# ElBaldo1/FastOptSolver

Measured on AMD Instinct MI355X. Metric: fista_iterations_per_second, higher is better.
Workload: dtype f32

## Files before the change

### fastoptsolver_amd/csrc/cluster_pass.hpp

```cpp
#pragma once
#include "batch_trial.hpp"

namespace fos {

constexpr int CP_ROWS = 16;
constexpr int CP_W = 1024;
constexpr int CP_ASTRIDE = CP_W + 4;
constexpr int CP_THREADS = 320;
constexpr int CP_SLOTS = 4;
constexpr int CP_FLAG_STRIDE = 32;
constexpr unsigned CP_SPIN_LIMIT = 1u << 18;
constexpr size_t CP_LDS_BYTES = (size_t)2 * CP_ROWS * CP_ASTRIDE * 4 + 4 * 64 * 16 + 2 * 64 * 16 + 16;

typedef unsigned long long cp_u64;
__device__ inline void cp_store_sc1(cp_u64* p, cp_u64 v) { __hip_atomic_store(p, v, __ATOMIC_RELAXED, __HIP_MEMORY_SCOPE_AGENT); }
__device__ inline cp_u64 cp_load_sc1(const cp_u64* p) { return __hip_atomic_load(p, __ATOMIC_RELAXED, __HIP_MEMORY_SCOPE_AGENT); }
__device__ inline cp_u64 cp_pack(float lo, float hi) { return ((cp_u64)__float_as_uint(hi) << 32) | __float_as_uint(lo); }

template <int CS, int MODE = 0>
__global__ __launch_bounds__(CP_THREADS) void cluster_pass_kernel(const float* __restrict__ A, int64_t lda,
                                                                 const float* __restrict__ b, int64_t m, int n, int n_pad,
                                                                 const float* __restrict__ xp, int64_t rows_per_cluster,
                                                                 int xcd_aware, float* __restrict__ xchg,
                                                                 unsigned* __restrict__ flags, unsigned epoch,
                                                                 float* __restrict__ slabs, int64_t n_stride,
                                                                 int* __restrict__ error) {
  extern __shared__ __attribute__((aligned(16))) char cp_lds[];
  float (*a_s)[CP_ROWS][CP_ASTRIDE] = reinterpret_cast<float (*)[CP_ROWS][CP_ASTRIDE]>(cp_lds);
  f32x4 (*red)[64] = reinterpret_cast<f32x4 (*)[64]>(cp_lds + (size_t)2 * CP_ROWS * CP_ASTRIDE * 4);
  f32x4 (*r_s)[64] = reinterpret_cast<f32x4 (*)[64]>(cp_lds + (size_t)2 * CP_ROWS * CP_ASTRIDE * 4 + 4 * 64 * 16);
  int* abort_s = reinterpret_cast<int*>(cp_lds + (size_t)2 * CP_ROWS * CP_ASTRIDE * 4 + 4 * 64 * 16 + 2 * 64 * 16);

  const int tid = threadIdx.x, lane = tid & 63, wave = tid >> 6;
  const bool mc = wave < 4;
  int cluster, member;
  if (xcd_aware) {
    const int xcd = blockIdx.x % 8, idx = blockIdx.x / 8;
    cluster = xcd + 8 * (idx / CS);
    member = idx % CS;
  } else {
    cluster = blockIdx.x / CS;
    member = blockIdx.x % CS;
  }
  const int col_strip = member * CP_W;
  const int64_t row_lo = (int64_t)cluster * rows_per_cluster;
  const int npanels = (int)(rows_per_cluster / CP_ROWS);
  if (tid == 0) *abort_s = 0;

  f32x4 xr[16];
  f32x4 G[16];
  f32x4 areg[CP_ROWS];
  const int wcol = col_strip + 256 * (wave & 3);
  if (mc) {
#pragma unroll
    for (int s = 0; s < 16; ++s) {
      const int col = wcol + 16 * s;
      const f32x4 v = *reinterpret_cast<const f32x4*>(xp + ((int64_t)((col < n_pad ? col : 0) / 16) * 4 + (lane >> 4)) * 64 +
                                                      (lane & 15) * 4);
      xr[s] = col < n_pad ? v : f32x4{0.f, 0.f, 0.f, 0.f};
      G[s] = f32x4{0.f, 0.f, 0.f, 0.f};
    }
  }
  int lcol = col_strip + 4 * tid;
  if (lcol >= n) lcol = n - 4;
  auto load_tile = [&](int pnl) {
    if ((MODE & 4) && pnl >= 2) return;
    if (pnl >= npanels) pnl = npanels - 1;
#pragma unroll
    for (int u = 0; u < CP_ROWS; ++u) {
      int64_t row = row_lo + (int64_t)pnl * CP_ROWS + u;
      if (row >= m) row = m - 1;
      areg[u] = __builtin_nontemporal_load(reinterpret_cast<const f32x4*>(A + row * lda + lcol));
    }
  };
  auto store_tile = [&](int buf) {
#pragma unroll
    for (int u = 0; u < CP_ROWS; ++u) *reinterpret_cast<f32x4*>(&a_s[buf][u][4 * tid]) = areg[u];
  };

  if (mc) {
    load_tile(0);
    store_tile(0);
    load_tile(1);
  }
  __syncthreads();

  for (int i = 0; i <= npanels; ++i) {
    if (mc) {
      if (i < npanels) {
        const int buf = i & 1;
        f32x4 acc = {0.f, 0.f, 0.f, 0.f}, acc_odd = {0.f, 0.f, 0.f, 0.f};
#pragma unroll
        for (int s = 0; s < ((MODE & 2) ? 1 : 16); ++s) {
          const f32x4 a4 = *reinterpret_cast<const f32x4*>(&a_s[buf][lane & 15][256 * wave + 16 * s + 4 * (lane >> 4)]);
          acc = __builtin_amdgcn_mfma_f32_16x16x4f32(a4.x, xr[s].x, acc, 0, 0, 0);
          acc_odd = __builtin_amdgcn_mfma_f32_16x16x4f32(a4.y, xr[s].y, acc_odd, 0, 0, 0);
          acc = __builtin_amdgcn_mfma_f32_16x16x4f32(a4.z, xr[s].z, acc, 0, 0, 0);
          acc_odd = __builtin_amdgcn_mfma_f32_16x16x4f32(a4.w, xr[s].w, acc_odd, 0, 0, 0);
        }
        red[wave][lane] = acc + acc_odd;
      }
    } else if (i >= 1 && (MODE & 1)) {
      r_s[(i - 1) & 1][lane] = red[0][lane];
    } else if (i >= 1) {
      const int q = i - 1;
      bool ok = true;
      if (lane < CS) {
        const unsigned* f = flags + ((size_t)cluster * CS + lane) * CP_FLAG_STRIDE;
        unsigned spins = 0;
        while ((int)(__hip_atomic_load(f, __ATOMIC_RELAXED, __HIP_MEMORY_SCOPE_AGENT) - epoch) < q + 1) {
          if (++spins > CP_SPIN_LIMIT) { ok = false; break; }
          __builtin_amdgcn_s_sleep(1);
        }
      }
      if (__ballot(!ok) != 0) {
        if (lane == 0) { *abort_s = 1; *error = 1; }
      } else {
        constexpr int GC = CS < 8 ? CS : 8;
        f32x4 r = {0.f, 0.f, 0.f, 0.f};
#pragma unroll 1
        for (int j0 = 0; j0 < CS; j0 += GC) {
          cp_u64 lo[GC], hi[GC];
#pragma unroll
          for (int j = 0; j < GC; ++j) {
            const cp_u64* src = reinterpret_cast<const cp_u64*>(
                xchg + (((size_t)cluster * CP_SLOTS + (q % CP_SLOTS)) * CS + j0 + j) * 256 + lane * 4);
            lo[j] = cp_load_sc1(src);
            hi[j] = cp_load_sc1(src + 1);
          }
#pragma unroll
          for (int j = 0; j < GC; ++j) {
            r.x += __uint_as_float((unsigned)lo[j]); r.y += __uint_as_float((unsigned)(lo[j] >> 32));
            r.z += __uint_as_float((unsigned)hi[j]); r.w += __uint_as_float((unsigned)(hi[j] >> 32));
          }
        }
        const int64_t row0 = row_lo + (int64_t)q * CP_ROWS + 4 * (lane >> 4);
        float rv[4] = {r.x, r.y, r.z, r.w};
#pragma unroll
        for (int c = 0; c < 4; ++c) {
          const int64_t row = row0 + c;
          rv[c] = row < m ? (b != nullptr ? rv[c] - b[row] : rv[c]) : 0.f;
        }
        r_s[q & 1][lane] = f32x4{rv[0], rv[1], rv[2], rv[3]};
      }
    }
    __syncthreads();
    if (*abort_s) break;
    if (mc) {
      if (i >= 1) {
        const int buf = (i - 1) & 1;
        const f32x4 r4 = r_s[(i - 1) & 1][lane];
        const float rc[4] = {r4.x, r4.y, r4.z, r4.w};
#pragma unroll
        for (int c = 0; c < ((MODE & 2) ? 1 : 4); ++c) {
#pragma unroll
          for (int t = 0; t < 16; ++t)
            G[t] = __builtin_amdgcn_mfma_f32_16x16x4f32(rc[c], a_s[buf][4 * (lane >> 4) + c][256 * wave + 16 * t + (lane & 15)],
                                                        G[t], 0, 0, 0);
        }
      }
    } else if (i < npanels && !(MODE & 1)) {
      const f32x4 s = ((red[0][lane] + red[1][lane]) + red[2][lane]) + red[3][lane];
      cp_u64* dst = reinterpret_cast<cp_u64*>(xchg + (((size_t)cluster * CP_SLOTS + (i % CP_SLOTS)) * CS + member) * 256 + lane * 4);
      cp_store_sc1(dst, cp_pack(s.x, s.y));
      cp_store_sc1(dst + 1, cp_pack(s.z, s.w));
      asm volatile("s_waitcnt vmcnt(0)" ::: "memory");
      if (lane == 0)
        __hip_atomic_store(flags + ((size_t)cluster * CS + member) * CP_FLAG_STRIDE, epoch + (unsigned)i + 1u, __ATOMIC_RELAXED,
                           __HIP_MEMORY_SCOPE_AGENT);
    }
    __syncthreads();
    if (mc && i + 1 < npanels) {
      store_tile((i + 1) & 1);
      load_tile(i + 2);
    }
    __syncthreads();
  }

  if (mc && *abort_s == 0) {
#pragma unroll
    for (int t = 0; t < 16; ++t) {
      const int col = wcol + 16 * t + (lane & 15);
      if (col < n) {
        const float gv[4] = {G[t].x, G[t].y, G[t].z, G[t].w};
#pragma unroll
        for (int r = 0; r < 4; ++r) slabs[((int64_t)cluster * BT_NV + 4 * (lane >> 4) + r) * n_stride + col] = gv[r];
      }
    }
  }
}

}
```

### fastoptsolver_amd/csrc/fos_internal.hpp

```cpp
#pragma once
#include <hip/hip_runtime.h>

#include <algorithm>
#include <atomic>
#include <cmath>
#include <cstdio>
#include <cstring>
#include <memory>
#include <string>
#include <chrono>
#include <vector>

#pragma GCC visibility push(default)
#include "../../include/fos.h"
#pragma GCC visibility pop
#include "batch_trial.hpp"
#include "cluster_pass.hpp"
#include "comm.hpp"
#include "gemv_multi.hpp"
#include "gemv_pair.hpp"
#include "gemv_tall.hpp"
#include "gemv_wide.hpp"
#include "gram_batch.hpp"
#include "gram_batch_dd.hpp"
// ... 4 lines not shown
#include "resident_batch.hpp"


namespace fosapi {

extern thread_local std::string g_err;

inline int fail(int code, const std::string& msg) {
  g_err = msg;
  return code;
}
#define HIP_TRY(expr)                                                                                   \
  do {                                                                                                  \
    hipError_t e_ = (expr);                                                                             \
    if (e_ != hipSuccess)                                                                               \
      return fail(FOS_ERR_HIP, std::string(#expr) + ": " + hipGetErrorString(e_));                      \
  } while (0)
#define LAUNCH_CHECK()                                                                                  \
  do {                                                                                                  \
    hipError_t e_ = hipGetLastError();                                                                  \
    if (e_ != hipSuccess) return fail(FOS_ERR_HIP, std::string("kernel launch: ") + hipGetErrorString(e_)); \
  } while (0)

template <class T, bool PINNED = false>
class DevBuf {
 public:
  DevBuf() = default;
  DevBuf(DevBuf&& o) noexcept : ptr_(o.ptr_), bytes_(o.bytes_) { o.ptr_ = nullptr; o.bytes_ = 0; }
  DevBuf& operator=(DevBuf&& o) noexcept {
    if (this != &o) {
      reset();
      std::swap(ptr_, o.ptr_);
      std::swap(bytes_, o.bytes_);
    }
    return *this;
  }
  ~DevBuf() { reset(); }
  void reset() {
    if (ptr_) (void)(PINNED ? hipHostFree(ptr_) : hipFree(ptr_));
    ptr_ = nullptr;
    bytes_ = 0;
  }
  int reserve(size_t count) {
    const size_t need = count * sizeof(T);
    if (ptr_ && need <= bytes_) return FOS_OK;
    reset();
    const hipError_t e = PINNED ? hipHostMalloc(&ptr_, need) : hipMalloc(&ptr_, need);
    if (e != hipSuccess) {
      ptr_ = nullptr;
      return fail(FOS_ERR_HIP, std::string(PINNED ? "hipHostMalloc(" : "hipMalloc(") + std::to_string(need) + " bytes): " +
                                   hipGetErrorString(e));
    }
    bytes_ = need;
    return FOS_OK;
  }
  T* get() const { return ptr_; }
  operator T*() const { return ptr_; }
  T* operator->() const { return ptr_; }

 private:
  T* ptr_ = nullptr;
  size_t bytes_ = 0;
};
template <class T>
using PinnedBuf = DevBuf<T, true>;

using fos::YSource;

typedef void (*FusedLaunch)(const void* A, int64_t lda, const float* b, int64_t m, int n, YSource ys, int64_t rpw,
                            float* slabs, double* rr_part, double* rr2_part, int nwg, hipStream_t st);

typedef void (*FusedLaunchDD)(const void* A, int64_t lda, const float* b, int64_t m, int n, YSource ys, int64_t rpw,
                              double* slabs, double* rr_part, int nwg, hipStream_t st);
struct MenuEntry {
  int dtype, threads, k, r;
  FusedLaunch with_g, resid_only, dual;
  FusedLaunchDD dd;
  FusedLaunch with_g_cb = nullptr, resid_only_cb = nullptr;
  FusedLaunch with_g_il = nullptr, resid_only_il = nullptr, dual_il = nullptr;
};
struct DdEntry { int dtype, threads, k, r; FusedLaunchDD fn; FusedLaunchDD fn_il = nullptr; };
typedef void (*MultiLaunch)(const float* A, int64_t lda, const float* b, int64_t m, int n, fos::MultiY ys, int64_t rpw,
                            float* slabs, double* rr_part, int nwg, hipStream_t st);
}

using fosapi::MenuEntry;
using fosapi::DdEntry;

using fosapi::DevBuf;
using fosapi::PinnedBuf;

struct LbfgsWork {
  int64_t n = 0;
  DevBuf<double> g, g_old, d, x_old, S, Y, vl;
  PinnedBuf<double> host;
  DevBuf<unsigned long long> t_start;
  double ticks_per_ms = 1e5;
  bool pass_stamps = false;
};

struct LbfgsMultiWork {
  int64_t n = 0;
  DevBuf<double> g;
  DevBuf<double> d, x_old, S, Y, vl, rr;
  PinnedBuf<double> host;
  DevBuf<unsigned> count;
  DevBuf<unsigned long long> t_start;
  double ticks_per_ms = 1e5;
};


struct PassPlan {
  int path = 0;
  bool resident = false;
  bool tall = false;
  bool colblock = false;
  int64_t cb_width = 0;
  int64_t slab_stride = 0;
  bool vec4 = false;
  const MenuEntry* entry = nullptr;
  int nwg = 0;
  int nslabs = 0;
  int64_t rows_per_wg = 0;
  int resid_grid = 0;
  DevBuf<float> slabs;
  DevBuf<double> rr_part;
  DevBuf<double> rr2_part;
  DevBuf<double> rvec;
  DevBuf<float> rneg;
  DevBuf<float> zeros;
  void reset() { *this = PassPlan{}; }
};

struct DdPlan {
  bool planned = false;
  const DdEntry* entry = nullptr;
  int nwg = 0;
  int64_t rows_per_wg = 0;
  int two_pass_chunks = 0;
  DevBuf<double> slabs;
  DevBuf<double> rr;
  void reset() { *this = DdPlan{}; }
};

struct MultiPlan {
  bool planned = false;
  int64_t panel_rows = 0;
  int gram_splits = 0;
  int64_t gram_rows_per_split = 0;
  int cp_cs = 0, cp_clusters = 0;
  int64_t cp_rows_per_cluster = 0;
  DevBuf<float> rbuf16;
  DevBuf<float> slabs16;
  DevBuf<float> cp_xchg;
  DevBuf<unsigned> cp_flags;
  DevBuf<int> cp_error;
  void reset() { *this = MultiPlan{}; }
};

struct DdMultiPlan {
  bool planned = false;
  int64_t n_pad = 0, panel_rows = 0, rows_per_split = 0;
  int splits = 0;
  DevBuf<double> xd;
  DevBuf<double> rdd;
  DevBuf<double> slabs;
  DevBuf<double> q_part;
  void reset() { *this = DdMultiPlan{}; }
};

struct CandPlan {
  bool planned = false;
  int64_t n_pad = 0;
  DevBuf<float> xp;
  DevBuf<double> q_part;
  DevBuf<double> bt_out;
  void reset() { *this = CandPlan{}; }
};

struct Scratch {
  DevBuf<float> gbuf_own;
  DevBuf<float> ybuf;
  DevBuf<double> dscal;
  DevBuf<double> part;
  DevBuf<double> lhist;
  DevBuf<float> rcols16;
  DevBuf<float> b16;
  DevBuf<double> mfold;
  DevBuf<double> cr_part;
  DevBuf<unsigned> cr_bar;
  DevBuf<unsigned> fz_bar;
  DevBuf<double> fz_part;
  DevBuf<double> fz_beta;
};

struct fos_problem {
  const void* A = nullptr;
  const float* b = nullptr;
  float* gbuf = nullptr;
  unsigned long long* fz_stamps = nullptr;
  fos_comm* comm = nullptr;
  int64_t m = 0, n = 0, lda = 0;
  int dtype = FOS_F32;
  int loss = FOS_LOSS_SQUARED;
  const float* row_weight = nullptr;
  hipStream_t stream = nullptr;
  int ncu = 256;
  bool col_sharded = false;
  unsigned plan_flags = 0;
  bool allow_resident = true;
  bool il = false;
  int dd_nwg_hint = 0;
  int cp_mode = 0;
  int chip_mode = 0;
  bool fused_on = false;
  unsigned cp_epoch = 1;
  PassPlan pass;
  DdPlan dd;
  MultiPlan multi;
  DdMultiPlan dm;
  CandPlan cand;
  Scratch ws;
  std::unique_ptr<LbfgsWork> lbfgs;
  std::unique_ptr<LbfgsMultiWork> lbfgs_multi;
  int profiling = 0;
  int64_t prof_seq = 0;
  bool prof_open = false;
  std::vector<hipEvent_t> ev_pool;
  size_t ev_used = 0;
  double prof_ms = 0.0;
  int64_t prof_launches = 0;
};

struct fos_fista {
  fos_problem* p = nullptr;
  fos::FistaParams prm{};
  bool host_valid = false;
  double h_t = 1.0, h_beta = 0.0;
  long long h_k = 0;
  DevBuf<double> part2;
  DevBuf<float> ynext;
  bool y_valid = false;
  bool pending = false;
  long long plain_count = 0;
  DevBuf<double> x_cur, x_prev;
  DevBuf<float> dlt;
  DevBuf<fos::FistaScalars> scal;
  bool precise = false;
  DevBuf<double> folded;
  bool tau_on_device = false;
  double* gbuf64 = nullptr;
  DevBuf<double> gbuf64_own;
  DevBuf<double> out5;
  int nupd = 0;
};

namespace fosapi {

const MenuEntry* wide_entry(int dtype);
const MenuEntry* find_entry(int dtype, int threads, int k, int r);
const MenuEntry* default_entry(int dtype, int64_t n);
int epc_of(int dtype);
int grid_1d(int64_t n, int per_block, int cap);
void plan_fused(fos_problem* p, const MenuEntry* e, int nwg_hint);
void apply_plan(fos_problem* p, unsigned flags);
enum PlanInput : unsigned {
  IN_PLAN = 1,
  IN_TUNE = 2,
  IN_TUNE_DD = 4,
  IN_COMM = 8,
  IN_CLUSTER = 16,
};
int invalidate(fos_problem* p, unsigned changed);
int plan_multi_mfma(fos_problem* p);
int ensure_workspace(fos_problem* p);
int ensure_batch_workspace(fos_problem* p);
int ensure_dd(fos_problem* p);
int prof_drain(fos_problem* p);
int prof_mark(fos_problem* p, bool start);
int aligned_vec(fos_problem* p, const float* v, const float** out);
bool batch_supported(const fos_problem* p);
MultiLaunch find_multi(int64_t n, int nv, bool bblock = false);
int pack_candidates(fos_problem* p, const float* X, int nv);
int stage_b16(fos_problem* p, const float* B, int64_t ldb, int nv);
int launch_pass(fos_problem* p, const YSource& ys, const float* b, bool with_g, int* n_rr, bool dual = false,
                double* rr_to = nullptr);
int launch_slab_reduce(fos_problem* p, int n_rr, float* gbuf, double* rr_out, const int* stopped);
int launch_batch_product(fos_problem* p, const void* A, const float* b, int64_t rows_total, int use_b, float* rout, int* nwg_out,
                         const int* stopped = nullptr, bool bblock = false);
bool fold_held_block(const int32_t* held, int nv, fos::FoldHeld* out);
int launch_batch_product_folds(fos_problem* p, const void* A, const float* b, int64_t rows_total, float* rout, int* nwg_out,
                               const uint8_t* fold_of_row, const fos::FoldHeld& held);
int launch_batch_product_logit(fos_problem* p, const void* A, const float* b, int64_t rows_total, float* rout, int* nwg_out,
                               const uint8_t* fold_of_row, const fos::FoldHeld* held);
int launch_batch_product_weighted(fos_problem* p, const void* A, const float* b, int use_b, int64_t rows_total, float* rout,
                                  int* nwg_out, const uint8_t* fold_of_row, const fos::FoldHeld* held, const float* row_weight);
int need_squared(const fos_problem* p, const char* fn);
int launch_residual_batch(fos_problem* p, int use_b, double* out16, const int* stopped = nullptr, const float* b16 = nullptr);
int launch_cluster_pass(fos_problem* p);
int launch_pass_dd(fos_problem* p, const YSource& ys, double alpha2, const double* l2vec, double* out);
int gemv_pair_dd_stamped(fos_problem* p, const double* x, double alpha2, double* grad_rr, unsigned long long* t_stamp, bool* stamped);
int dd_pass_stamps(fos_problem* p, bool* yes);
bool pair_dd_multi_supported(const fos_problem* p);
int pair_dd_multi(fos_problem* p, const fos::DdMultiCols& c, int ncols, unsigned live, double alpha2, const float* b16);
int comm_allreduce(fos_comm* c, void* buf, size_t count, bool f64, hipStream_t st);
int reduce_across(fos_problem* p, void* buf, size_t count, bool f64);

inline int check_batch_items(const char* fn, const fos_batch_item* items, int count, int64_t ld) {
// ... 14 lines not shown
```

### fastoptsolver_amd/csrc/fos_plan.hip

```cpp
#include "fos_internal.hpp"

namespace fosapi {

thread_local std::string g_err;



template <typename T, int THREADS, int K, int R, int MINW, bool WITH_G, int NBUF, bool DUAL, bool DRAIN = false, bool CB = false,
          bool IL = false>
void fused_launch(const void* A, int64_t lda, const float* b, int64_t m, int n, YSource ys, int64_t rpw, float* slabs,
                  double* rr_part, double* rr2_part, int nwg, hipStream_t st) {
  hipLaunchKernelGGL((fos::gemv_pair_kernel<T, THREADS, K, R, true, MINW, WITH_G, NBUF, IL, DUAL, DRAIN, float, false, CB>), dim3(nwg),
                     dim3(THREADS), 0, st, reinterpret_cast<const T*>(A), lda, b, m, n, ys, rpw, slabs, rr_part,
                     rr2_part);
}


template <typename K>
int raise_dynamic_lds(K kernel, size_t bytes, std::atomic<uint64_t>& done) {
  int dev = 0;
  if (hipGetDevice(&dev) != hipSuccess) return FOS_ERR_HIP;
  const uint64_t bit = 1ull << (dev & 63);
  if (done.load(std::memory_order_acquire) & bit) return FOS_OK;
  if (hipFuncSetAttribute(reinterpret_cast<const void*>(kernel), hipFuncAttributeMaxDynamicSharedMemorySize, (int)bytes) !=
// ... 765 lines not shown
constexpr int DM_P1_PER_CU = 2;
int ensure_dd_multi(fos_problem* p) {
  if (p->dm.planned) return FOS_OK;
  const int64_t n = p->n;
  p->dm.n_pad = (n + fos::DM_COLS - 1) / fos::DM_COLS * fos::DM_COLS;
  p->dm.panel_rows = std::min<int64_t>(256 * (int64_t)p->ncu, (p->m + 255) / 256 * 256);
  const int64_t strips = (n + fos::DM_COLS - 1) / fos::DM_COLS;
  int64_t splits = std::max<int64_t>(1, (2 * (int64_t)p->ncu + strips - 1) / strips);
  splits = std::min<int64_t>(splits, std::max<int64_t>(1, p->dm.panel_rows / 256));
  p->dm.rows_per_split = ((p->dm.panel_rows + splits - 1) / splits + fos::DM_ROWS - 1) / fos::DM_ROWS * fos::DM_ROWS;
  p->dm.splits = (int)((p->dm.panel_rows + p->dm.rows_per_split - 1) / p->dm.rows_per_split);
  const int64_t panels = (p->m + p->dm.panel_rows - 1) / p->dm.panel_rows;
  int rc;
  if ((rc = p->dm.xd.reserve((size_t)p->dm.n_pad * fos::BT_NV)) || (rc = p->dm.rdd.reserve((size_t)p->dm.panel_rows * fos::BT_NV)) ||
      (rc = p->dm.slabs.reserve((size_t)p->dm.splits * fos::BT_NV * n)) ||
      (rc = p->dm.q_part.reserve((size_t)panels * DM_P1_PER_CU * p->ncu * fos::BT_NV)))
    return rc;
  p->dm.planned = true;
  return FOS_OK;
}

template <typename T>
int run_pair_dd_multi(fos_problem* p, const fos::DdMultiCols& c, int ncols, unsigned live, double alpha2, const float* b16) {
  const int64_t n = p->n, esz = sizeof(T);
  hipLaunchKernelGGL(fos::xd_pack_kernel, dim3(grid_1d(p->dm.n_pad * fos::BT_NV, 256, 4 * p->ncu)), dim3(256), 0, p->stream, c,
                     live, (int)n, (int)p->dm.n_pad, p->dm.xd);
  LAUNCH_CHECK();
  const int64_t strips = (n + fos::DM_COLS - 1) / fos::DM_COLS;
  int64_t nparts = 0;
  int rc;
  for (int64_t row0 = 0, panel = 0; row0 < p->m; row0 += p->dm.panel_rows, ++panel) {
    const int64_t rows = std::min<int64_t>(p->dm.panel_rows, p->m - row0);
    const T* Ap = reinterpret_cast<const T*>(reinterpret_cast<const char*>(p->A) + (size_t)row0 * p->lda * esz);
    const int64_t ngroups = (rows + fos::DM_ROWS - 1) / fos::DM_ROWS;
    int64_t nwg = std::min<int64_t>(ngroups, DM_P1_PER_CU * (int64_t)p->ncu);
    const int64_t gpw = (ngroups + nwg - 1) / nwg;
    nwg = (ngroups + gpw - 1) / gpw;
    if ((rc = prof_mark(p, true))) return rc;
    hipLaunchKernelGGL(fos::residual_dd_mfma_kernel<T>, dim3((unsigned)nwg), dim3(fos::DM_THREADS), 0, p->stream, Ap, p->lda,
                       b16 + row0 * fos::BT_NV, rows, (int)n, (const double*)p->dm.xd, gpw, p->dm.q_part + nparts * fos::BT_NV,
                       p->dm.rdd);
    LAUNCH_CHECK();
    if ((rc = prof_mark(p, false))) return rc;
    nparts += nwg;
    const dim3 grid((unsigned)strips, (unsigned)p->dm.splits);
    if ((rc = prof_mark(p, true))) return rc;
    if (panel)
      hipLaunchKernelGGL((fos::gram_dd_mfma_kernel<T, true>), grid, dim3(fos::DM_THREADS), 0, p->stream, Ap, p->lda, rows,
                         (int)n, (const double*)p->dm.rdd, p->dm.rows_per_split, p->dm.slabs, n);
    else
      hipLaunchKernelGGL((fos::gram_dd_mfma_kernel<T, false>), grid, dim3(fos::DM_THREADS), 0, p->stream, Ap, p->lda, rows,
                         (int)n, (const double*)p->dm.rdd, p->dm.rows_per_split, p->dm.slabs, n);
    LAUNCH_CHECK();
    if ((rc = prof_mark(p, false))) return rc;
  }
  hipLaunchKernelGGL(fos::pair_dd_multi_finish_kernel, dim3(grid_1d(n, 256, 64), ncols), dim3(256), 0, p->stream,
                     (const double*)p->dm.slabs, p->dm.splits, (int)n, (const double*)p->dm.q_part, (int)nparts, alpha2, c);
  LAUNCH_CHECK();
  return FOS_OK;
}

typedef int (*PairDdMultiRun)(fos_problem*, const fos::DdMultiCols&, int, unsigned, double, const float*);
struct PairDdMultiEntry { int dtype; PairDdMultiRun run; };
const PairDdMultiEntry kPairDdMulti[] = {
    {FOS_F32, run_pair_dd_multi<float>},
    {FOS_BF16, run_pair_dd_multi<fos::bf16_t>},
};

int pair_dd_multi(fos_problem* p, const fos::DdMultiCols& c, int ncols, unsigned live, double alpha2, const float* b16) {
  if (!pair_dd_multi_supported(p))
    return fail(FOS_ERR_UNSUPPORTED, "fos_gemv_pair_dd_multi: no matrix-core pair for this shape (needs the aligned streaming "
                                     "layout, 65..16384 columns, unsharded)");
  if (ncols < 1) return FOS_OK;
  int rc = ensure_dd_multi(p);
  if (rc) return rc;
  for (const auto& e : kPairDdMulti)
    if (e.dtype == p->dtype) return e.run(p, c, ncols, live, alpha2, b16);
  return fail(FOS_ERR_UNSUPPORTED, "fos_gemv_pair_dd_multi: storage type not served");
}

int aligned_vec(fos_problem* p, const float* v, const float** out) {
  if ((reinterpret_cast<uintptr_t>(v) & 15u) == 0) {
    *out = v;
    return FOS_OK;
  }
  HIP_TRY(hipMemcpyAsync(p->ws.ybuf, v, (size_t)p->n * sizeof(float), hipMemcpyDeviceToDevice, p->stream));
  *out = p->ws.ybuf;
  return FOS_OK;
}

bool il_default(const fos_problem* p) {
  const int64_t bytes = p->m * p->n * (p->dtype == FOS_F32 ? 4 : 2);
  return bytes >= (12ll << 30);
}

bool vec_layout(const fos_problem* p) {
  const int epc = epc_of(p->dtype);
  return (p->n % epc == 0) && (p->lda % epc == 0) && ((reinterpret_cast<uintptr_t>(p->A) & 15u) == 0);
}
void plan_resident(fos_problem* p) { p->pass.resident = fos::resident_fits(p->m, p->n) && p->allow_resident && p->comm == nullptr; }
const MenuEntry* colblock_entry(const fos_problem* p, int64_t* width) {
  const int64_t cap = 16384, blocks = (p->n + cap - 1) / cap;
  *width = ((p->n + blocks - 1) / blocks + 63) / 64 * 64;
  const MenuEntry* ce = default_entry(p->dtype, *width);
  return ce && ce->with_g_cb && ce->resid_only_cb ? ce : nullptr;
}
void plan_colblock(fos_problem* p, const MenuEntry* ce, int64_t width) {
  plan_fused(p, ce, 0);
  p->pass.colblock = true;
  p->pass.cb_width = width;
}

void apply_plan(fos_problem* p, unsigned flags) {
  const int64_t n = p->n;
  p->plan_flags = flags;
  p->pass.vec4 = (n % 4 == 0);
  p->allow_resident = !(flags & FOS_PLAN_NO_RESIDENT);
  p->il = (flags & FOS_PLAN_INTERLEAVE) ? true : (flags & FOS_PLAN_NO_INTERLEAVE) ? false : il_default(p);
  plan_resident(p);
  const bool vec_ok = vec_layout(p);
  int64_t cb_width = 0;
  const MenuEntry* e = vec_ok ? default_entry(p->dtype, n) : nullptr;
  if ((n <= fos::TL_MAX_N || (n <= tlr_max_n(p->dtype) && vec_ok)) && !(flags & FOS_PLAN_NO_TALL))
    plan_tall(p, tall_entry(p->dtype, n, p->lda, p->A));
  else if (e) plan_fused(p, e, 0);
  else if (vec_ok && n <= fos::WD_MAX_N && !(flags & FOS_PLAN_NO_WIDE)) plan_fused(p, wide_entry(p->dtype), 0);
  else if (const MenuEntry* ce = (vec_ok && !(flags & FOS_PLAN_NO_COLBLOCK)) ? colblock_entry(p, &cb_width) : nullptr)
    plan_colblock(p, ce, cb_width);
  else plan_fallback(p);
}

int invalidate(fos_problem* p, unsigned changed) {
  if (changed & (IN_TUNE_DD | IN_CLUSTER)) HIP_TRY(hipStreamSynchronize(p->stream));
  if (changed & IN_PLAN) p->pass.reset();
  if (changed & IN_COMM) plan_resident(p);
  if (changed & (IN_PLAN | IN_TUNE | IN_TUNE_DD | IN_COMM)) p->dd.reset();
  if (changed & (IN_PLAN | IN_COMM | IN_CLUSTER)) p->multi.reset();
  return FOS_OK;
}

int plan_multi_mfma(fos_problem* p) {
  if (p->multi.planned) return FOS_OK;
  int rc;
  const bool is_bf16 = p->dtype == FOS_BF16;
  const int cs_need = (int)((p->n + fos::CP_W - 1) / fos::CP_W);
  const bool cluster_wins = (p->n == 4096 || p->n == 8192) && p->m * p->n >= (1ll << 29) && !p->comm;
  const bool want_cluster = p->cp_mode == 1 || (p->cp_mode == 0 && cluster_wins);
  if (want_cluster && !is_bf16 && p->ncu % 8 == 0) {
    const int cs = cs_need <= 2 ? 0 : cs_need <= 4 ? 4 : cs_need <= 8 ? 8 : cs_need <= 16 ? 16 : 0;
    if (cs && (p->ncu / 8) % cs == 0 && p->m >= (int64_t)(p->ncu / cs) * fos::CP_ROWS * 8) {
      p->multi.cp_cs = cs;
      p->multi.cp_clusters = p->ncu / cs;
      p->multi.cp_rows_per_cluster = ((p->m + p->multi.cp_clusters - 1) / p->multi.cp_clusters + fos::CP_ROWS - 1) / fos::CP_ROWS * fos::CP_ROWS;
      if ((rc = p->multi.cp_xchg.reserve((size_t)p->ncu * fos::CP_SLOTS * 256)) ||
          (rc = p->multi.cp_flags.reserve((size_t)p->ncu * fos::CP_FLAG_STRIDE)) || (rc = p->multi.cp_error.reserve(1)))
        return rc;
      HIP_TRY(hipMemsetAsync(p->multi.cp_flags, 0, (size_t)p->ncu * fos::CP_FLAG_STRIDE * sizeof(unsigned), p->stream));
      HIP_TRY(hipMemsetAsync(p->multi.cp_error, 0, sizeof(int), p->stream));
    }
  }
  const int64_t rows = 256 * (int64_t)p->ncu;
  p->multi.panel_rows = std::min<int64_t>(rows, (p->m + 255) / 256 * 256);
  if (p->col_sharded && p->comm->kind != 0) {
    const int64_t fit = (int64_t)(p->comm->cap_bytes / (fos::BT_NV * sizeof(float))) / 256 * 256;
    if (fit < 256) return fail(FOS_ERR_ARG, "fos_fista_run_multi: the communicator's inbox rows hold less than one 256-row "
                                            "panel of 16 residual columns (16 KiB)");
    p->multi.panel_rows = std::min<int64_t>(p->multi.panel_rows, fit);
  }
  const int64_t strips = (p->n + (is_bf16 ? fos::GQ_COLS : fos::GB_COLS) - 1) / (is_bf16 ? fos::GQ_COLS : fos::GB_COLS);
  int64_t splits = std::max<int64_t>(1, (2 * (int64_t)p->ncu + strips - 1) / strips);
  splits = std::min<int64_t>(splits, std::max<int64_t>(1, p->multi.panel_rows / 256));
  p->multi.gram_rows_per_split = ((p->multi.panel_rows + splits - 1) / splits + fos::GB_ROWS - 1) / fos::GB_ROWS * fos::GB_ROWS;
  p->multi.gram_splits = (int)((p->multi.panel_rows + p->multi.gram_rows_per_split - 1) / p->multi.gram_rows_per_split);
  if (p->multi.cp_cs) p->multi.gram_splits = p->multi.cp_clusters;
  if ((rc = p->multi.rbuf16.reserve((size_t)p->multi.panel_rows * fos::BT_NV)) ||
      (rc = p->multi.slabs16.reserve((size_t)p->multi.gram_splits * fos::BT_NV * p->n)))
    return rc;
  p->multi.planned = true;
  return FOS_OK;
}

int ensure_dd(fos_problem* p) {
  if (p->dd.planned || p->pass.resident) return FOS_OK;
  int rc;
  int nslabs = 0;
  int64_t stride = p->n;
  int n_rr = 0;
  if (p->pass.tall) {
    nslabs = p->pass.nwg; stride = p->pass.slab_stride; n_rr = p->pass.nwg;
  } else {
    const DdEntry* e = nullptr;
    if (p->pass.path == 0 && !p->col_sharded)
      for (const auto& c : kDdMenu)
        if (c.dtype == p->dtype && (int64_t)c.threads * c.k * epc_of(p->dtype) >= p->n) { e = &c; break; }
    if (e) {
      p->dd.entry = e;
      const int64_t cap = (int64_t)e->threads * e->k * epc_of(p->dtype);
      const bool full = p->n * 10 > 9 * cap, sparse = p->n * 10 <= 7 * cap;
      int nwg = p->ncu * (e->threads >= 512 ? 1
                          : e->threads == 256 ? (e->k == 1 ? 4 : (e->k == 2 && sparse ? 4 : 2))
                                              : (e->k >= 3 || (e->k == 2 && full) ? 4 : 8));
      const int64_t row_bytes = p->n * (p->dtype == FOS_F32 ? 4 : 2);
      if (e->threads == 64 && p->m * row_bytes < (512ll << 20)) nwg = std::min(nwg, 4 * p->ncu);
      const int64_t min_rows = std::max<int64_t>(2 * (int64_t)e->r, (65536 + row_bytes - 1) / row_bytes);
      if (p->dd_nwg_hint > 0) nwg = p->dd_nwg_hint;
      if (p->m < (int64_t)nwg * min_rows) nwg = (int)std::max<int64_t>(1, p->m / min_rows);
      p->dd.rows_per_wg = (p->m + nwg - 1) / nwg;
      p->dd.nwg = (int)((p->m + p->dd.rows_per_wg - 1) / p->dd.rows_per_wg);
      nslabs = p->dd.nwg; n_rr = p->dd.nwg;
    } else {
      const int chunks = (int)std::max<int64_t>(1, std::min<int64_t>(64, p->m / 64));
      p->dd.rows_per_wg = (p->m + chunks - 1) / chunks;
      p->dd.two_pass_chunks = (int)((p->m + p->dd.rows_per_wg - 1) / p->dd.rows_per_wg);
      p->dd.nwg = (int)std::max<int64_t>(1, std::min<int64_t>(2048, (p->m + 3) / 4));
      nslabs = p->dd.two_pass_chunks; n_rr = p->dd.nwg;
      if ((rc = p->pass.rvec.reserve(p->m))) return rc;
    }
  }
  if ((rc = p->dd.rr.reserve(std::max(n_rr, 1))) || (rc = p->dd.slabs.reserve((size_t)nslabs * stride))) return rc;
  p->dd.planned = true;
  return FOS_OK;
}

template <int CS>
int launch_cluster_pass_cs(fos_problem* p) {
  auto kern = fos::cluster_pass_kernel<CS>;
  static std::atomic<uint64_t> done{0};
  if (raise_dynamic_lds(kern, fos::CP_LDS_BYTES, done)) return fail(FOS_ERR_HIP, "cluster pass: dynamic LDS size refused");
  const float* A = (const float*)p->A;
  int64_t lda = p->lda, m = p->m, rpc = p->multi.cp_rows_per_cluster, n_stride = p->n;
  int n = (int)p->n, n_pad = (int)p->cand.n_pad, xcd_aware = 1;
  const float* b = p->b;
  const float* xp = p->cand.xp;
  unsigned epoch = p->cp_epoch;
  hipLaunchKernelGGL(kern, dim3((unsigned)(p->multi.cp_clusters * CS)), dim3(fos::CP_THREADS), (unsigned)fos::CP_LDS_BYTES, p->stream, A,
                     lda, b, m, n, n_pad, xp, rpc, xcd_aware, p->multi.cp_xchg, p->multi.cp_flags, epoch, p->multi.slabs16, n_stride, p->multi.cp_error);
  LAUNCH_CHECK();
  p->cp_epoch += (unsigned)(rpc / fos::CP_ROWS) + 16u;
  return FOS_OK;
}
int launch_cluster_pass(fos_problem* p) {
  switch (p->multi.cp_cs) {
    case 4: return launch_cluster_pass_cs<4>(p);
    case 8: return launch_cluster_pass_cs<8>(p);
    case 16: return launch_cluster_pass_cs<16>(p);
  }
  return fail(FOS_ERR_STATE, "cluster pass: no plan");
}


template <int ORDER>
__global__ __launch_bounds__(512) void stream_read_kernel(const fos::f32x4* __restrict__ src, size_t n16, float* __restrict__ sink) {
  constexpr int UNR = 8, THREADS = 512;
  constexpr bool BLOCKS = ORDER == 0;
  fos::f32x4 acc = {0.f, 0.f, 0.f, 0.f};
  if constexpr (ORDER == 2) {
    constexpr size_t CH = (size_t)UNR * THREADS;
    size_t base = (size_t)blockIdx.x * CH;
    for (; base + CH <= n16; base += (size_t)gridDim.x * CH) {
      fos::f32x4 v[UNR];
#pragma unroll
      for (int u = 0; u < UNR; ++u) v[u] = __builtin_nontemporal_load(src + base + threadIdx.x + (size_t)u * THREADS);
#pragma unroll
      for (int u = 0; u < UNR; ++u) acc += v[u];
    }
    for (size_t i = base + threadIdx.x; i < n16 && i < base + CH; i += THREADS) acc += __builtin_nontemporal_load(src + i);
  } else if constexpr (BLOCKS) {
    const size_t per = ((n16 + gridDim.x - 1) / gridDim.x + THREADS * UNR - 1) / (THREADS * UNR) * (THREADS * UNR);
    const size_t lo = per * blockIdx.x, hi = lo + per < n16 ? lo + per : n16;
    size_t i = lo + threadIdx.x;
    for (; i + (size_t)(UNR - 1) * THREADS < hi; i += (size_t)UNR * THREADS) {
      fos::f32x4 v[UNR];
#pragma unroll
      for (int u = 0; u < UNR; ++u) v[u] = __builtin_nontemporal_load(src + i + (size_t)u * THREADS);
#pragma unroll
      for (int u = 0; u < UNR; ++u) acc += v[u];
    }
    for (; i < hi; i += THREADS) acc += __builtin_nontemporal_load(src + i);
  } else {
    const size_t stride = (size_t)gridDim.x * THREADS;
    size_t i = (size_t)blockIdx.x * THREADS + threadIdx.x;
    for (; i + (UNR - 1) * stride < n16; i += UNR * stride) {
      fos::f32x4 v[UNR];
#pragma unroll
      for (int u = 0; u < UNR; ++u) v[u] = __builtin_nontemporal_load(src + i + u * stride);
#pragma unroll
      for (int u = 0; u < UNR; ++u) acc += v[u];
    }
    for (; i < n16; i += stride) acc += __builtin_nontemporal_load(src + i);
  }
  const float t = fos::wave_sum((acc.x + acc.y) + (acc.z + acc.w));
  if ((threadIdx.x & 63) == 0) sink[blockIdx.x * 8 + (threadIdx.x >> 6)] = t;
}

}

using namespace fosapi;

extern "C" {

const char* fos_last_error(void) { return g_err.c_str(); }
int fos_abi_version(void) { return FOS_ABI_VERSION; }

int fos_problem_create(fos_problem** out, const void* A, int64_t m, int64_t n, int64_t lda, int a_dtype,
                       const float* b, void* stream) {
  if (!out || !A || m <= 0 || n <= 0 || lda < n) return fail(FOS_ERR_ARG, "fos_problem_create: bad shape/pointer");
  if (a_dtype != FOS_F32 && a_dtype != FOS_BF16) return fail(FOS_ERR_ARG, "fos_problem_create: bad a_dtype");
  if (n > (int64_t)1 << 30) return fail(FOS_ERR_ARG, "fos_problem_create: n too large");
  fos_problem* p = new fos_problem();
  p->A = A; p->b = b; p->m = m; p->n = n; p->lda = lda; p->dtype = a_dtype;
  p->stream = reinterpret_cast<hipStream_t>(stream);
  int dev = 0;
  hipDeviceProp_t prop;
  if (hipGetDevice(&dev) != hipSuccess || hipGetDeviceProperties(&prop, dev) != hipSuccess) {
    delete p;
    return fail(FOS_ERR_HIP, "fos_problem_create: no HIP device");
  }
  p->ncu = prop.multiProcessorCount;
  apply_plan(p, 0);
  int rc;
  if ((rc = ensure_workspace(p)) || (rc = p->ws.gbuf_own.reserve(n + 4)) || (rc = p->ws.ybuf.reserve(n)) ||
      (rc = p->ws.dscal.reserve(256)) || (rc = p->ws.part.reserve(std::max<size_t>(1024, (n + fos::RCOLS - 1) / fos::RCOLS) * 4))) {
    delete p;
    return rc;
  }
  p->gbuf = p->ws.gbuf_own;
  *out = p;
  return FOS_OK;
}

int fos_problem_set_loss(fos_problem* p, int loss) {
  if (!p) return fail(FOS_ERR_ARG, "fos_problem_set_loss: null");
  if (loss != FOS_LOSS_SQUARED && loss != FOS_LOSS_LOGISTIC) return fail(FOS_ERR_ARG, "fos_problem_set_loss: unknown loss");
  if (loss == FOS_LOSS_LOGISTIC) {
    if (!p->b) return fail(FOS_ERR_UNSUPPORTED, "fos_problem_set_loss: a logistic problem needs b (the labels)");
    if (p->comm || p->col_sharded) return fail(FOS_ERR_UNSUPPORTED, "fos_problem_set_loss: sharded problems are not served");
    if (!pair_dd_multi_supported(p))
      return fail(FOS_ERR_UNSUPPORTED, "fos_problem_set_loss: the logistic loss runs on the matrix-core pair (aligned streaming "
                                       "layout, 65..16384 columns)");
  }
  p->loss = loss;
  return FOS_OK;
}

int fos_problem_get_loss(const fos_problem* p, int* loss) {
  if (!p || !loss) return fail(FOS_ERR_ARG, "fos_problem_get_loss: null");
  *loss = p->loss;
  return FOS_OK;
}

int fos_row_weights_bind(const float* w, fos_problem* p) {
  if (!p) return fail(FOS_ERR_ARG, "fos_row_weights_bind: null problem");
  if (((uintptr_t)w & 15) != 0) return fail(FOS_ERR_ARG, "fos_row_weights_bind: the weights are not 16-byte aligned");
  if (w) {
    if (!p->b) return fail(FOS_ERR_UNSUPPORTED, "fos_row_weights_bind: a weighted problem needs b");
    if (p->comm || p->col_sharded) return fail(FOS_ERR_UNSUPPORTED, "fos_row_weights_bind: sharded problems are not served");
    if (!pair_dd_multi_supported(p))
      return fail(FOS_ERR_UNSUPPORTED, "fos_row_weights_bind: row weights run on the matrix-core pair (aligned streaming layout, "
                                       "65..16384 columns)");
  }
  p->row_weight = w;
  return FOS_OK;
}

int fos_row_weights_get(const float** w_out, const fos_problem* p) {
  if (!p || !w_out) return fail(FOS_ERR_ARG, "fos_row_weights_get: null");
  *w_out = p->row_weight;
  return FOS_OK;
}

int fos_problem_set_comm(fos_problem* p, fos_comm* c) {
  if (!p) return fail(FOS_ERR_ARG, "fos_problem_set_comm: null");
  if (int rc_ = need_squared(p, "fos_problem_set_comm")) return rc_;
  p->comm = c;
  return invalidate(p, IN_COMM);
}

int fos_problem_set_comm_cols(fos_problem* p, fos_comm* c) {
  if (!p || !c) return fail(FOS_ERR_ARG, "fos_problem_set_comm_cols: null");
  if (int rc_ = need_squared(p, "fos_problem_set_comm_cols")) return rc_;
  if (!vec_layout(p) || p->n <= tlr_max_n(p->dtype))
    return fail(FOS_ERR_UNSUPPORTED, "fos_problem_set_comm_cols: needs the streaming layout (aligned, more than 32 chunks of 16 bytes per row and rank)");
  int64_t cb_width = 0;
  const MenuEntry* ce = colblock_entry(p, &cb_width);
  if (!ce) return fail(FOS_ERR_UNSUPPORTED, "fos_problem_set_comm_cols: no column-block kernel for this block width");
  p->comm = c;
  p->col_sharded = true;
  if (int rc = invalidate(p, IN_PLAN | IN_COMM)) return rc;
  p->pass.vec4 = true;
  plan_colblock(p, ce, cb_width);
  return ensure_workspace(p);
// ... 549 lines not shown
```

Measured before the change: 104.8.

## Replace flag-based cluster exchange with tagged self-validating ring and split wave roles

```diff
diff --git a/fastoptsolver_amd/csrc/cluster_pass.hpp b/fastoptsolver_amd/csrc/cluster_pass.hpp
--- a/fastoptsolver_amd/csrc/cluster_pass.hpp
+++ b/fastoptsolver_amd/csrc/cluster_pass.hpp
@@ -8,31 +8,31 @@
 constexpr int CP_ASTRIDE = CP_W + 4;
 constexpr int CP_THREADS = 320;
 constexpr int CP_SLOTS = 4;
-constexpr int CP_FLAG_STRIDE = 32;
+constexpr int CP_WORDS = 256;
 constexpr unsigned CP_SPIN_LIMIT = 1u << 18;
-constexpr size_t CP_LDS_BYTES = (size_t)2 * CP_ROWS * CP_ASTRIDE * 4 + 4 * 64 * 16 + 2 * 64 * 16 + 16;
+constexpr size_t CP_LDS_BYTES = (size_t)2 * CP_ROWS * CP_ASTRIDE * 4 + 2 * 4 * 64 * 16 + 2 * 64 * 16 + 16;
 
 typedef unsigned long long cp_u64;
 __device__ inline void cp_store_sc1(cp_u64* p, cp_u64 v) { __hip_atomic_store(p, v, __ATOMIC_RELAXED, __HIP_MEMORY_SCOPE_AGENT); }
 __device__ inline cp_u64 cp_load_sc1(const cp_u64* p) { return __hip_atomic_load(p, __ATOMIC_RELAXED, __HIP_MEMORY_SCOPE_AGENT); }
-__device__ inline cp_u64 cp_pack(float lo, float hi) { return ((cp_u64)__float_as_uint(hi) << 32) | __float_as_uint(lo); }
+__device__ inline cp_u64 cp_pack(float value, unsigned tag) { return ((cp_u64)tag << 32) | __float_as_uint(value); }
+__device__ inline bool cp_arrived(cp_u64 w, unsigned epoch, int q) { return (int)((unsigned)(w >> 32) - epoch) >= q + 1; }
 
 template <int CS, int MODE = 0>
 __global__ __launch_bounds__(CP_THREADS) void cluster_pass_kernel(const float* __restrict__ A, int64_t lda,
                                                                  const float* __restrict__ b, int64_t m, int n, int n_pad,
                                                                  const float* __restrict__ xp, int64_t rows_per_cluster,
-                                                                 int xcd_aware, float* __restrict__ xchg,
-                                                                 unsigned* __restrict__ flags, unsigned epoch,
+                                                                 int xcd_aware, cp_u64* __restrict__ ring, unsigned epoch,
                                                                  float* __restrict__ slabs, int64_t n_stride,
                                                                  int* __restrict__ error) {
   extern __shared__ __attribute__((aligned(16))) char cp_lds[];
   float (*a_s)[CP_ROWS][CP_ASTRIDE] = reinterpret_cast<float (*)[CP_ROWS][CP_ASTRIDE]>(cp_lds);
-  f32x4 (*red)[64] = reinterpret_cast<f32x4 (*)[64]>(cp_lds + (size_t)2 * CP_ROWS * CP_ASTRIDE * 4);
-  f32x4 (*r_s)[64] = reinterpret_cast<f32x4 (*)[64]>(cp_lds + (size_t)2 * CP_ROWS * CP_ASTRIDE * 4 + 4 * 64 * 16);
-  int* abort_s = reinterpret_cast<int*>(cp_lds + (size_t)2 * CP_ROWS * CP_ASTRIDE * 4 + 4 * 64 * 16 + 2 * 64 * 16);
-
-  const int tid = threadIdx.x, lane = tid & 63, wave = tid >> 6;
-  const bool mc = wave < 4;
+  f32x4 (*red)[4][64] = reinterpret_cast<f32x4 (*)[4][64]>(cp_lds + (size_t)2 * CP_ROWS * CP_ASTRIDE * 4);
+  f32x4 (*r_s)[64] = reinterpret_cast<f32x4 (*)[64]>(cp_lds + (size_t)2 * CP_ROWS * CP_ASTRIDE * 4 + 2 * 4 * 64 * 16);
+  int* abort_s = reinterpret_cast<int*>(cp_lds + (size_t)2 * CP_ROWS * CP_ASTRIDE * 4 + 2 * 4 * 64 * 16 + 2 * 64 * 16);
+
+  const int tid = threadIdx.x, lane = tid & 63;
+  const int wave = __builtin_amdgcn_readfirstlane(tid >> 6);
   int cluster, member;
   if (xcd_aware) {
     const int xcd = blockIdx.x % 8, idx = blockIdx.x / 8;
@@ -47,11 +47,11 @@
   const int npanels = (int)(rows_per_cluster / CP_ROWS);
   if (tid == 0) *abort_s = 0;
 
-  f32x4 xr[16];
-  f32x4 G[16];
-  f32x4 areg[CP_ROWS];
-  const int wcol = col_strip + 256 * (wave & 3);
-  if (mc) {
+  if (wave < 4) {
+    f32x4 xr[16];
+    f32x4 G[16];
+    f32x4 areg[CP_ROWS];
+    const int wcol = col_strip + 256 * wave;
 #pragma unroll
     for (int s = 0; s < 16; ++s) {
       const int col = wcol + 16 * s;
@@ -60,131 +60,178 @@
       xr[s] = col < n_pad ? v : f32x4{0.f, 0.f, 0.f, 0.f};
       G[s] = f32x4{0.f, 0.f, 0.f, 0.f};
     }
-  }
-  int lcol = col_strip + 4 * tid;
-  if (lcol >= n) lcol = n - 4;
-  auto load_tile = [&](int pnl) {
-    if ((MODE & 4) && pnl >= 2) return;
-    if (pnl >= npanels) pnl = npanels - 1;
-#pragma unroll
-    for (int u = 0; u < CP_ROWS; ++u) {
-      int64_t row = row_lo + (int64_t)pnl * CP_ROWS + u;
-      if (row >= m) row = m - 1;
-      areg[u] = __builtin_nontemporal_load(reinterpret_cast<const f32x4*>(A + row * lda + lcol));
-    }
-  };
-  auto store_tile = [&](int buf) {
-#pragma unroll
-    for (int u = 0; u < CP_ROWS; ++u) *reinterpret_cast<f32x4*>(&a_s[buf][u][4 * tid]) = areg[u];
-  };
-
-  if (mc) {
+    int lcol = col_strip + 4 * tid;
+    if (lcol >= n) lcol = n - 4;
+    auto load_tile = [&](int pnl) {
+      if ((MODE & 4) && pnl >= 2) return;
+      if (pnl >= npanels) pnl = npanels - 1;
+#pragma unroll
+      for (int u = 0; u < CP_ROWS; ++u) {
+        int64_t row = row_lo + (int64_t)pnl * CP_ROWS + u;
+        if (row >= m) row = m - 1;
+        areg[u] = __builtin_nontemporal_load(reinterpret_cast<const f32x4*>(A + row * lda + lcol));
+      }
+    };
+    auto store_tile = [&](int buf) {
+#pragma unroll
+      for (int u = 0; u < CP_ROWS; ++u) *reinterpret_cast<f32x4*>(&a_s[buf][u][4 * tid]) = areg[u];
+    };
     load_tile(0);
     store_tile(0);
     load_tile(1);
-  }
-  __syncthreads();
-
-  for (int i = 0; i <= npanels; ++i) {
-    if (mc) {
+    __syncthreads();
+
+    for (int i = 0; i <= npanels; ++i) {
       if (i < npanels) {
         const int buf = i & 1;
         f32x4 acc = {0.f, 0.f, 0.f, 0.f}, acc_odd = {0.f, 0.f, 0.f, 0.f};
-#pragma unroll
-        for (int s = 0; s < ((MODE & 2) ? 1 : 16); ++s) {
-          const f32x4 a4 = *reinterpret_cast<const f32x4*>(&a_s[buf][lane & 15][256 * wave + 16 * s + 4 * (lane >> 4)]);
-          acc = __builtin_amdgcn_mfma_f32_16x16x4f32(a4.x, xr[s].x, acc, 0, 0, 0);
-          acc_odd = __builtin_amdgcn_mfma_f32_16x16x4f32(a4.y, xr[s].y, acc_odd, 0, 0, 0);
-          acc = __builtin_amdgcn_mfma_f32_16x16x4f32(a4.z, xr[s].z, acc, 0, 0, 0);
-          acc_odd = __builtin_amdgcn_mfma_f32_16x16x4f32(a4.w, xr[s].w, acc_odd, 0, 0, 0);
-        }
-        red[wave][lane] = acc + acc_odd;
-      }
-    } else if (i >= 1 && (MODE & 1)) {
-      r_s[(i - 1) & 1][lane] = red[0][lane];
-    } else if (i >= 1) {
-      const int q = i - 1;
-      bool ok = true;
-      if (lane < CS) {
-        const unsigned* f = flags + ((size_t)cluster * CS + lane) * CP_FLAG_STRIDE;
-        unsigned spins = 0;
-        while ((int)(__hip_atomic_load(f, __ATOMIC_RELAXED, __HIP_MEMORY_SCOPE_AGENT) - epoch) < q + 1) {
-          if (++spins > CP_SPIN_LIMIT) { ok = false; break; }
-          __builtin_amdgcn_s_sleep(1);
-        }
-      }
-      if (__ballot(!ok) != 0) {
-        if (lane == 0) { *abort_s = 1; *error = 1; }
-      } else {
-        constexpr int GC = CS < 8 ? CS : 8;
-        f32x4 r = {0.f, 0.f, 0.f, 0.f};
-#pragma unroll 1
-        for (int j0 = 0; j0 < CS; j0 += GC) {
-          cp_u64 lo[GC], hi[GC];
-#pragma unroll
-          for (int j = 0; j < GC; ++j) {
-            const cp_u64* src = reinterpret_cast<const cp_u64*>(
-                xchg + (((size_t)cluster * CP_SLOTS + (q % CP_SLOTS)) * CS + j0 + j) * 256 + lane * 4);
-            lo[j] = cp_load_sc1(src);
-            hi[j] = cp_load_sc1(src + 1);
-          }
-#pragma unroll
-          for (int j = 0; j < GC; ++j) {
-            r.x += __uint_as_float((unsigned)lo[j]); r.y += __uint_as_float((unsigned)(lo[j] >> 32));
-            r.z += __uint_as_float((unsigned)hi[j]); r.w += __uint_as_float((unsigned)(hi[j] >> 32));
-          }
-        }
-        const int64_t row0 = row_lo + (int64_t)q * CP_ROWS + 4 * (lane >> 4);
-        float rv[4] = {r.x, r.y, r.z, r.w};
-#pragma unroll
-        for (int c = 0; c < 4; ++c) {
-          const int64_t row = row0 + c;
-          rv[c] = row < m ? (b != nullptr ? rv[c] - b[row] : rv[c]) : 0.f;
-        }
-        r_s[q & 1][lane] = f32x4{rv[0], rv[1], rv[2], rv[3]};
-      }
-    }
-    __syncthreads();
-    if (*abort_s) break;
-    if (mc) {
+        const float* a_row = &a_s[buf][lane & 15][256 * wave + 4 * (lane >> 4)];
+        if constexpr (!(MODE & 2)) {
+          f32x4 a4[2][4];
+#pragma unroll
+          for (int k = 0; k < 4; ++k) a4[0][k] = *reinterpret_cast<const f32x4*>(a_row + 16 * k);
+#pragma unroll
+          for (int s0 = 0; s0 < 16; s0 += 4) {
+            const int cur = (s0 >> 2) & 1;
+            if (s0 + 4 < 16) {
+#pragma unroll
+              for (int k = 0; k < 4; ++k) a4[cur ^ 1][k] = *reinterpret_cast<const f32x4*>(a_row + 16 * (s0 + 4 + k));
+            }
+            __builtin_amdgcn_sched_barrier(0);
+#pragma unroll
+            for (int k = 0; k < 4; ++k) {
+              const int s = s0 + k;
+              acc = __builtin_amdgcn_mfma_f32_16x16x4f32(a4[cur][k].x, xr[s].x, acc, 0, 0, 0);
+              acc_odd = __builtin_amdgcn_mfma_f32_16x16x4f32(a4[cur][k].y, xr[s].y, acc_odd, 0, 0, 0);
+              acc = __builtin_amdgcn_mfma_f32_16x16x4f32(a4[cur][k].z, xr[s].z, acc, 0, 0, 0);
+              acc_odd = __builtin_amdgcn_mfma_f32_16x16x4f32(a4[cur][k].w, xr[s].w, acc_odd, 0, 0, 0);
+            }
+            __builtin_amdgcn_sched_barrier(0);
+          }
+        } else {
+#pragma unroll
+          for (int s = 0; s < ((MODE & 2) ? 1 : 16); ++s) {
+            const f32x4 a4 = *reinterpret_cast<const f32x4*>(a_row + 16 * s);
+            acc = __builtin_amdgcn_mfma_f32_16x16x4f32(a4.x, xr[s].x, acc, 0, 0, 0);
+            acc_odd = __builtin_amdgcn_mfma_f32_16x16x4f32(a4.y, xr[s].y, acc_odd, 0, 0, 0);
+            acc = __builtin_amdgcn_mfma_f32_16x16x4f32(a4.z, xr[s].z, acc, 0, 0, 0);
+            acc_odd = __builtin_amdgcn_mfma_f32_16x16x4f32(a4.w, xr[s].w, acc_odd, 0, 0, 0);
+          }
+        }
+        red[i & 1][wave][lane] = acc + acc_odd;
+      }
+      __syncthreads();
+      if (*abort_s) break;
       if (i >= 1) {
         const int buf = (i - 1) & 1;
         const f32x4 r4 = r_s[(i - 1) & 1][lane];
         const float rc[4] = {r4.x, r4.y, r4.z, r4.w};
-#pragma unroll
-        for (int c = 0; c < ((MODE & 2) ? 1 : 4); ++c) {
-#pragma unroll
-          for (int t = 0; t < 16; ++t)
-            G[t] = __builtin_amdgcn_mfma_f32_16x16x4f32(rc[c], a_s[buf][4 * (lane >> 4) + c][256 * wave + 16 * t + (lane & 15)],
-                                                        G[t], 0, 0, 0);
-        }
-      }
-    } else if (i < npanels && !(MODE & 1)) {
-      const f32x4 s = ((red[0][lane] + red[1][lane]) + red[2][lane]) + red[3][lane];
-      cp_u64* dst = reinterpret_cast<cp_u64*>(xchg + (((size_t)cluster * CP_SLOTS + (i % CP_SLOTS)) * CS + member) * 256 + lane * 4);
-      cp_store_sc1(dst, cp_pack(s.x, s.y));
-      cp_store_sc1(dst + 1, cp_pack(s.z, s.w));
-      asm volatile("s_waitcnt vmcnt(0)" ::: "memory");
-      if (lane == 0)
-        __hip_atomic_store(flags + ((size_t)cluster * CS + member) * CP_FLAG_STRIDE, epoch + (unsigned)i + 1u, __ATOMIC_RELAXED,
-                           __HIP_MEMORY_SCOPE_AGENT);
-    }
+        const float* a_col = &a_s[buf][4 * (lane >> 4)][256 * wave + (lane & 15)];
+        if constexpr (!(MODE & 2)) {
+          float bv[2][16];
+#pragma unroll
+          for (int t = 0; t < 16; ++t) bv[0][t] = a_col[16 * t];
+#pragma unroll
+          for (int c = 0; c < 4; ++c) {
+            if (c + 1 < 4) {
+#pragma unroll
+              for (int t = 0; t < 16; ++t) bv[(c + 1) & 1][t] = a_col[(c + 1) * CP_ASTRIDE + 16 * t];
+            }
+            __builtin_amdgcn_sched_barrier(0);
+#pragma unroll
+            for (int t = 0; t < 16; ++t) G[t] = __builtin_amdgcn_mfma_f32_16x16x4f32(rc[c], bv[c & 1][t], G[t], 0, 0, 0);
+            __builtin_amdgcn_sched_barrier(0);
+          }
+        } else {
+#pragma unroll
+          for (int c = 0; c < ((MODE & 2) ? 1 : 4); ++c) {
+#pragma unroll
+            for (int t = 0; t < 16; ++t)
+              G[t] = __builtin_amdgcn_mfma_f32_16x16x4f32(rc[c], a_col[c * CP_ASTRIDE + 16 * t], G[t], 0, 0, 0);
+          }
+        }
+      }
+      if (i + 1 < npanels) {
+        store_tile((i + 1) & 1);
+        load_tile(i + 2);
+      }
+      __builtin_amdgcn_wave_barrier();
+    }
+
+    if (*abort_s == 0) {
+#pragma unroll
+      for (int t = 0; t < 16; ++t) {
+        const int col = wcol + 16 * t + (lane & 15);
+        if (col < n) {
+          const float gv[4] = {G[t].x, G[t].y, G[t].z, G[t].w};
+#pragma unroll
+          for (int r = 0; r < 4; ++r) slabs[((int64_t)cluster * BT_NV + 4 * (lane >> 4) + r) * n_stride + col] = gv[r];
+        }
+      }
+    }
+  } else {
     __syncthreads();
-    if (mc && i + 1 < npanels) {
-      store_tile((i + 1) & 1);
-      load_tile(i + 2);
-    }
-    __syncthreads();
-  }
-
-  if (mc && *abort_s == 0) {
-#pragma unroll
-    for (int t = 0; t < 16; ++t) {
-      const int col = wcol + 16 * t + (lane & 15);
-      if (col < n) {
-        const float gv[4] = {G[t].x, G[t].y, G[t].z, G[t].w};
-#pragma unroll
-        for (int r = 0; r < 4; ++r) slabs[((int64_t)cluster * BT_NV + 4 * (lane >> 4) + r) * n_stride + col] = gv[r];
+    for (int i = 0; i <= npanels; ++i) {
+      if (i >= 1 && (MODE & 1)) {
+        r_s[(i - 1) & 1][lane] = red[0][0][lane];
+      } else if (i >= 1) {
+        const int q = i - 1;
+        constexpr int GC = CS < 8 ? CS : 8;
+        bool ok = true;
+        unsigned spins = 0;
+        f32x4 r = {0.f, 0.f, 0.f, 0.f};
+#pragma unroll 1
+        for (int j0 = 0; j0 < CS && ok; j0 += GC) {
+          const cp_u64* src = ring + (((size_t)cluster * CP_SLOTS + (q % CP_SLOTS)) * CS + j0) * CP_WORDS + lane;
+          cp_u64 w[GC][4];
+#pragma unroll
+          for (int j = 0; j < GC; ++j)
+#pragma unroll
+            for (int c = 0; c < 4; ++c) w[j][c] = cp_load_sc1(src + j * CP_WORDS + c * 64);
+          for (;;) {
+            bool all = true;
+#pragma unroll
+            for (int j = 0; j < GC; ++j)
+#pragma unroll
+              for (int c = 0; c < 4; ++c) all &= cp_arrived(w[j][c], epoch, q);
+            if (__all(all)) break;
+            if (++spins > CP_SPIN_LIMIT) { ok = false; break; }
+            __builtin_amdgcn_s_sleep(2);
+#pragma unroll
+            for (int j = 0; j < GC; ++j)
+#pragma unroll
+              for (int c = 0; c < 4; ++c)
+                if (!cp_arrived(w[j][c], epoch, q)) w[j][c] = cp_load_sc1(src + j * CP_WORDS + c * 64);
+          }
+#pragma unroll
+          for (int j = 0; j < GC; ++j) {
+            r.x += __uint_as_float((unsigned)w[j][0]); r.y += __uint_as_float((unsigned)w[j][1]);
+            r.z += __uint_as_float((unsigned)w[j][2]); r.w += __uint_as_float((unsigned)w[j][3]);
+          }
+        }
+        if (!ok) {
+          if (lane == 0) { *abort_s = 1; *error = 1; }
+        } else {
+          const int64_t row0 = row_lo + (int64_t)q * CP_ROWS + 4 * (lane >> 4);
+          float rv[4] = {r.x, r.y, r.z, r.w};
+#pragma unroll
+          for (int c = 0; c < 4; ++c) {
+            const int64_t row = row0 + c;
+            rv[c] = row < m ? (b != nullptr ? rv[c] - b[row] : rv[c]) : 0.f;
+          }
+          r_s[q & 1][lane] = f32x4{rv[0], rv[1], rv[2], rv[3]};
+        }
+      }
+      __syncthreads();
+      if (*abort_s) break;
+      if (i < npanels && !(MODE & 1)) {
+        const f32x4 s = ((red[i & 1][0][lane] + red[i & 1][1][lane]) + red[i & 1][2][lane]) + red[i & 1][3][lane];
+        cp_u64* dst = ring + (((size_t)cluster * CP_SLOTS + (i % CP_SLOTS)) * CS + member) * CP_WORDS + lane;
+        const unsigned tag = epoch + (unsigned)i + 1u;
+        cp_store_sc1(dst, cp_pack(s.x, tag));
+        cp_store_sc1(dst + 64, cp_pack(s.y, tag));
+        cp_store_sc1(dst + 128, cp_pack(s.z, tag));
+        cp_store_sc1(dst + 192, cp_pack(s.w, tag));
       }
     }
   }
diff --git a/fastoptsolver_amd/csrc/fos_internal.hpp b/fastoptsolver_amd/csrc/fos_internal.hpp
--- a/fastoptsolver_amd/csrc/fos_internal.hpp
+++ b/fastoptsolver_amd/csrc/fos_internal.hpp
@@ -180,8 +180,7 @@
   int64_t cp_rows_per_cluster = 0;
   DevBuf<float> rbuf16;
   DevBuf<float> slabs16;
-  DevBuf<float> cp_xchg;
-  DevBuf<unsigned> cp_flags;
+  DevBuf<fos::cp_u64> cp_ring;
   DevBuf<int> cp_error;
   void reset() { *this = MultiPlan{}; }
 };
diff --git a/fastoptsolver_amd/csrc/fos_plan.hip b/fastoptsolver_amd/csrc/fos_plan.hip
--- a/fastoptsolver_amd/csrc/fos_plan.hip
+++ b/fastoptsolver_amd/csrc/fos_plan.hip
@@ -941,10 +941,9 @@
       p->multi.cp_cs = cs;
       p->multi.cp_clusters = p->ncu / cs;
       p->multi.cp_rows_per_cluster = ((p->m + p->multi.cp_clusters - 1) / p->multi.cp_clusters + fos::CP_ROWS - 1) / fos::CP_ROWS * fos::CP_ROWS;
-      if ((rc = p->multi.cp_xchg.reserve((size_t)p->ncu * fos::CP_SLOTS * 256)) ||
-          (rc = p->multi.cp_flags.reserve((size_t)p->ncu * fos::CP_FLAG_STRIDE)) || (rc = p->multi.cp_error.reserve(1)))
-        return rc;
-      HIP_TRY(hipMemsetAsync(p->multi.cp_flags, 0, (size_t)p->ncu * fos::CP_FLAG_STRIDE * sizeof(unsigned), p->stream));
+      const size_t ring_words = (size_t)p->ncu * fos::CP_SLOTS * fos::CP_WORDS;
+      if ((rc = p->multi.cp_ring.reserve(ring_words)) || (rc = p->multi.cp_error.reserve(1))) return rc;
+      HIP_TRY(hipMemsetAsync(p->multi.cp_ring, 0, ring_words * sizeof(fos::cp_u64), p->stream));
       HIP_TRY(hipMemsetAsync(p->multi.cp_error, 0, sizeof(int), p->stream));
     }
   }
@@ -1021,11 +1020,16 @@
   int n = (int)p->n, n_pad = (int)p->cand.n_pad, xcd_aware = 1;
   const float* b = p->b;
   const float* xp = p->cand.xp;
+  const unsigned advance = (unsigned)(rpc / fos::CP_ROWS) + 16u;
+  if (p->cp_epoch > (1u << 30) - advance) {
+    HIP_TRY(hipMemsetAsync(p->multi.cp_ring, 0, (size_t)p->ncu * fos::CP_SLOTS * fos::CP_WORDS * sizeof(fos::cp_u64), p->stream));
+    p->cp_epoch = 1;
+  }
   unsigned epoch = p->cp_epoch;
   hipLaunchKernelGGL(kern, dim3((unsigned)(p->multi.cp_clusters * CS)), dim3(fos::CP_THREADS), (unsigned)fos::CP_LDS_BYTES, p->stream, A,
-                     lda, b, m, n, n_pad, xp, rpc, xcd_aware, p->multi.cp_xchg, p->multi.cp_flags, epoch, p->multi.slabs16, n_stride, p->multi.cp_error);
-  LAUNCH_CHECK();
-  p->cp_epoch += (unsigned)(rpc / fos::CP_ROWS) + 16u;
+                     lda, b, m, n, n_pad, xp, rpc, xcd_aware, p->multi.cp_ring, epoch, p->multi.slabs16, n_stride, p->multi.cp_error);
+  LAUNCH_CHECK();
+  p->cp_epoch += advance;
   return FOS_OK;
 }
 int launch_cluster_pass(fos_problem* p) {
```

Result: no change. 104.7 (-0.1%).
